# ZhengyiLuo/PHC

Measured on NVIDIA H100. Metric: env-steps/sec (fused obs+reward+PPO) at 4096 envs/GPU, higher is better.
Workload: dtype f32

## Files before the change

### include/phc_b200.h

```cpp
#ifndef PHC_B200_H_
#define PHC_B200_H_

#include <stdint.h>

#ifdef __cplusplus
extern "C" {
#endif

#if defined(_WIN32)
#define PHC_API __declspec(dllexport)
#else
#define PHC_API __attribute__((visibility("default")))
#endif

#define PHC_OK 0
#define PHC_ERR_INVALID_ARG (-1)
#define PHC_ERR_UNSUPPORTED (-2)
#define PHC_ERR_CUDA (-3)

PHC_API int phc_version(void);
PHC_API const char* phc_last_error(void);
PHC_API int64_t phc_launch_count(void);
PHC_API int phc_compiled_sm(void);

// ... 203 lines not shown
#define PHC_ACT_RELU_BITS 4
#define PHC_ACT_MASK_BITS 5
PHC_API int phc_gemm(const float* A, int64_t lda, int32_t a_kmajor, const float* B, int64_t ldb, int32_t b_kmajor, float* C,
             int64_t ldc, int32_t M, int32_t N, int32_t K, float alpha, const float* bias, int32_t act,
             float* aux, int64_t ldaux, int32_t accumulate, int32_t k_splits, void* stream);
PHC_API int phc_split_tf32(const float* x, int64_t ldx, int64_t rows, int32_t cols, float* hi, float* lo, int64_t ldo, void* stream);
PHC_API int phc_gemm_tc5(const float* A_hi, const float* A_lo, int64_t lda, int32_t a_kmajor, const float* B_hi, const float* B_lo,
                 int64_t ldb, int32_t b_kmajor, float* C, float* C_hi ,
                 float* C_lo, int64_t ldc, int32_t M, int32_t N, int32_t K, float alpha, const float* bias, int32_t act,
                 float* aux, int64_t ldaux, int32_t accumulate, int32_t k_splits, void* stream);
#define PHC_GEMM_GROUP_MAX 8
typedef struct PhcGemmDesc {
  const float* A; int64_t lda; int32_t a_kmajor;
  const float* B; int64_t ldb; int32_t b_kmajor;
  float* C; int64_t ldc;
  int32_t M, N, K;
  float alpha;
  const float* bias;
  int32_t act;
  float* aux; int64_t ldaux;
  int32_t accumulate, k_splits;
  const float* B_lo;
  const float* B_img;
} PhcGemmDesc;
typedef struct PhcGemmImageDesc {
  const float* B; int64_t ldb; int32_t b_kmajor;
  int32_t N, K;
  float* img;
} PhcGemmImageDesc;
PHC_API int64_t phc_gemm_image_floats(int32_t N, int32_t K);
PHC_API int phc_gemm_make_images(const PhcGemmImageDesc* images, int32_t count, void* stream);
PHC_API int phc_split_lo(const float* x, float* lo, int64_t n, void* stream);
PHC_API int phc_gemm_group(const PhcGemmDesc* problems, int32_t count, void* stream);
PHC_API int phc_gemm_tc5s(const float* A, int64_t lda, int32_t a_kmajor, const float* B, int64_t ldb, int32_t b_kmajor, float* C,
                  int64_t ldc, int32_t M, int32_t N, int32_t K, float alpha, const float* bias, int32_t act,
                  float* aux, int64_t ldaux, int32_t accumulate, int32_t k_splits, void* stream);
#define PHC_GEMM_FP32_3XTF32 0
#define PHC_GEMM_TF32_SINGLE_PASS 1
PHC_API int phc_gemm_set_precision(int32_t mode);
PHC_API int phc_gemm_tc5s_set_ctas(int32_t ctas);
PHC_API int phc_gemm_tc5s_set_tile(int32_t width);
PHC_API int phc_gemm_tc5s_set_sched(int32_t mode);
PHC_API int phc_pd_targets(const float* actions, int64_t lda, int64_t n, int32_t num_dofs, int32_t num_actions,
                   const int32_t* dof_of_action, const float* offset, const float* scale, const uint8_t* zero_mask,
                   float* out, int64_t ldo, void* stream);
PHC_API int phc_colsum(const float* X, int64_t ld, int32_t M, int32_t N, float alpha, float* out, int32_t accumulate,
// ... 45 lines not shown
```

### phc_b200/_lib.py

```python
from __future__ import annotations

import ctypes as C
import os

_HERE = os.path.dirname(os.path.abspath(__file__))
LIB_PATH = os.environ.get("PHC_LIB_PATH") or os.path.join(_HERE, "lib", "libphc_b200.so")

PHC_FLAG_UPRIGHT = 1 << 0
PHC_FLAG_LOCAL_ROOT_OBS = 1 << 1
PHC_FLAG_ROOT_HEIGHT_OBS = 1 << 2
PHC_FLAG_POWER_REWARD = 1 << 3
PHC_FLAG_EARLY_TERM = 1 << 4
PHC_FLAG_NO_COLLISION = 1 << 5
PHC_FLAG_TERM_USE_MEAN = 1 << 6
PHC_FLAG_OBS_ONLY = 1 << 7
PHC_FLAG_REWARD_FROM_CACHE = 1 << 8
PHC_FLAG_ZERO_OUT_FAR = 1 << 9
PHC_FLAG_CYCLE_MOTION = 1 << 10
PHC_FLAG_NO_SPECIALISE = 1 << 11
PHC_FLAG_SUBSET_REWARD = 1 << 12
PHC_FLAG_TASK_OBS_KP = 1 << 13
PHC_FLAG_RECOVERY = 1 << 14
PHC_FLAG_AMP_CURRENT = 1 << 15
PHC_ACT_NONE, PHC_ACT_RELU, PHC_ACT_SILU, PHC_ACT_SILU_BWD, PHC_ACT_RELU_BITS, PHC_ACT_MASK_BITS = 0, 1, 2, 3, 4, 5
# ... 30 lines not shown
        ("num_envs", C.c_int32), ("time_steps", C.c_int32), ("dt", C.c_float), ("traj_dt", C.c_float),
        ("flags", C.c_uint32),
        ("k_pos", C.c_float), ("k_rot", C.c_float), ("k_vel", C.c_float), ("k_ang_vel", C.c_float),
        ("w_pos", C.c_float), ("w_rot", C.c_float), ("w_vel", C.c_float), ("w_ang_vel", C.c_float),
        ("power_coef", C.c_float), ("term_thresh", C.c_float * PHC_MAX_BODIES), ("term_dist_mean", C.c_float),
        ("ext_parent", C.c_int32 * PHC_MAX_EXT_BODIES), ("ext_pos", (C.c_float * 3) * PHC_MAX_EXT_BODIES),
        ("num_key_bodies", C.c_int32), ("key_bodies", C.c_int32 * PHC_MAX_KEY_BODIES),
        ("amp_joints", C.c_int32 * PHC_MAX_AMP_JOINTS), ("num_amp_joints", C.c_int32),
        ("obs", _p), ("obs_stride", C.c_int64), ("rew", _p), ("reward_raw", _p), ("reset", _p), ("terminate", _p),
        ("amp_out", _p), ("amp_hist_in", _p), ("amp_out_stride", C.c_int64), ("amp_steps", C.c_int32),
        ("ref_body_pos", _p), ("ref_body_rot", _p), ("ref_body_vel", _p), ("ref_body_ang_vel", _p),
        ("ref_cache", _p),
        ("close_distance", C.c_float), ("far_distance", C.c_float), ("max_episode_length", C.c_int32), ("point_goal", _p),
        ("cycle_phase", _p), ("mpjpe", _p), ("body_pos_gt", _p), ("ring_head", _p),
        ("num_track", C.c_int32), ("track_slot", C.c_int8 * PHC_MAX_BODIES), ("occlusion", _p), ("shape_params", _p), ("num_shape", C.c_int32),
        ("limb_weights", _p), ("num_limb", C.c_int32), ("recovery_counter", _p),
    ]


class PhcGemmDesc(C.Structure):
    _fields_ = [("A", _p), ("lda", C.c_int64), ("a_kmajor", C.c_int32), ("B", _p), ("ldb", C.c_int64), ("b_kmajor", C.c_int32),
                ("C", _p), ("ldc", C.c_int64), ("M", C.c_int32), ("N", C.c_int32), ("K", C.c_int32), ("alpha", C.c_float),
                ("bias", _p), ("act", C.c_int32), ("aux", _p), ("ldaux", C.c_int64), ("accumulate", C.c_int32), ("k_splits", C.c_int32),
                ("B_lo", _p), ("B_img", _p)]


class PhcGemmImageDesc(C.Structure):
    _fields_ = [("B", _p), ("ldb", C.c_int64), ("b_kmajor", C.c_int32), ("N", C.c_int32), ("K", C.c_int32), ("img", _p)]


class PhcColsumDesc(C.Structure):
    _fields_ = [("X", _p), ("ld", C.c_int64), ("M", C.c_int32), ("N", C.c_int32), ("alpha", C.c_float), ("out", _p)]


PHC_GEMM_GROUP_MAX = 8
PHC_GEMM_FP32_3XTF32, PHC_GEMM_TF32_SINGLE_PASS = 0, 1

SIGNATURES = {
    "phc_version": (C.c_int, []),
    "phc_last_error": (C.c_char_p, []),
    "phc_compiled_sm": (C.c_int, []),
    "phc_launch_count": (C.c_int64, []),
    "phc_env_motion_gather": (C.c_int, [C.POINTER(PhcMotionLib), _p, C.c_int64, _p, _p]),
    "phc_motion_body_stride": (C.c_int, [C.c_int32]),
    "phc_reset_bookkeeping": (C.c_int, [_p, _p, _p, C.c_int64, _p, _p, _p, _p, _p, _p, _p, _p]),
    "phc_motion_dof_stride": (C.c_int, [C.c_int32]),
    "phc_motion_pack_dofs": (C.c_int, [_p, _p, C.c_int64, C.c_int32, _p, _p]),
# ... 91 lines not shown
```

### phc_b200/csrc/gemm_wgmma.cu

```cuda
#include <cuda_runtime.h>
#include <stdint.h>
#include <stdlib.h>
#include <string.h>

#include <type_traits>

#include "../../include/phc_b200.h"
#include "phc_common.cuh"

extern "C" void phc_set_error(const char* msg);
extern "C" int phc_check_cuda(cudaError_t e, const char* what);
extern "C" void phc_count_launches(int n);

namespace phc {
namespace wg {

constexpr int BM = 128, NUM_THREADS = 256, MAX_PROBLEMS = PHC_GEMM_GROUP_MAX;

template <int BN>
struct Cfg {
  static constexpr int BK = BN == 128 ? 32 : 16;
  static constexpr int A_TILE = BM * BK * 4;
  static constexpr int B_TILE = BN * BK * 4;
  static constexpr int STAGE = 2 * (A_TILE + B_TILE);
  static constexpr int STAGES = 3;
  static constexpr int SMEM = STAGES * STAGE;
  static constexpr int SBO = BK * 32;
  static constexpr int A_PER = BM * BK / NUM_THREADS;
  static constexpr int B_PER = BN * BK / NUM_THREADS;
};

constexpr int IMG_ROWS = 128, IMG_BK = 32, IMG_HALF = IMG_ROWS * IMG_BK, IMG_BLOCK = 2 * IMG_HALF;
constexpr int IMG_STAGES = 4;

struct Prob {
  const float* A; const float* B; const float* A_lo; const float* B_lo;
  const float* B_img;
  float* C; float* C_hi; float* C_lo;
  const float* bias;
  float* aux;
  long long lda, ldb, ldc, ldaux;
  int M, N, K;
  float alpha;
  int act, accumulate, a_k, b_k, k_splits;
  int tiles_m, tiles_n, kb_total, kb_per, tile_begin, tile_count;
  unsigned int* turn;
  int turn_first, turn_total;
};

struct Params {
  Prob p[MAX_PROBLEMS];
  int count, total_tiles;
  unsigned int* sched;
};

__device__ __forceinline__ void wgmma_tf32_n128(float (&d)[64], uint64_t da, uint64_t db) {
  asm volatile(
      "{\n\t.reg .pred p;\n\tsetp.ne.b32 p, 1, 0;\n\t"
      "wgmma.mma_async.sync.aligned.m64n128k8.f32.tf32.tf32 {%0, %1, %2, %3, %4, %5, %6, %7, %8, %9, %10, %11, %12, %13, %14, %15, %16, %17, %18, %19, %20, %21, %22, %23, %24, %25, %26, %27, %28, %29, %30, %31, %32, %33, %34, %35, %36, %37, %38, %39, %40, %41, %42, %43, %44, %45, %46, %47, %48, %49, %50, %51, %52, %53, %54, %55, %56, %57, %58, %59, %60, %61, %62, %63}, %64, %65, p, 1, 1;\n\t}"
      : "+f"(d[0]), "+f"(d[1]), "+f"(d[2]), "+f"(d[3]), "+f"(d[4]), "+f"(d[5]), "+f"(d[6]), "+f"(d[7]), "+f"(d[8]), "+f"(d[9]), "+f"(d[10]), "+f"(d[11]), "+f"(d[12]), "+f"(d[13]), "+f"(d[14]), "+f"(d[15]), "+f"(d[16]), "+f"(d[17]), "+f"(d[18]), "+f"(d[19]), "+f"(d[20]), "+f"(d[21]), "+f"(d[22]), "+f"(d[23]), "+f"(d[24]), "+f"(d[25]), "+f"(d[26]), "+f"(d[27]), "+f"(d[28]), "+f"(d[29]), "+f"(d[30]), "+f"(d[31]), "+f"(d[32]), "+f"(d[33]), "+f"(d[34]), "+f"(d[35]), "+f"(d[36]), "+f"(d[37]), "+f"(d[38]), "+f"(d[39]), "+f"(d[40]), "+f"(d[41]), "+f"(d[42]), "+f"(d[43]), "+f"(d[44]), "+f"(d[45]), "+f"(d[46]), "+f"(d[47]), "+f"(d[48]), "+f"(d[49]), "+f"(d[50]), "+f"(d[51]), "+f"(d[52]), "+f"(d[53]), "+f"(d[54]), "+f"(d[55]), "+f"(d[56]), "+f"(d[57]), "+f"(d[58]), "+f"(d[59]), "+f"(d[60]), "+f"(d[61]), "+f"(d[62]), "+f"(d[63])
// ... 140 lines not shown
        sts32(s_hi + o, hi(u[j]));
        if (MODE == 0) sts32(s_lo + o, split_lo(u[j]));
        if (MODE == 2) sts32(s_lo + o, ul[j]);
      }
    }
  }
}

__device__ __forceinline__ void split_rna(float x, float& h, float& l) {
  uint32_t a, b;
  asm("cvt.rna.tf32.f32 %0, %1;" : "=r"(a) : "f"(x));
  const float res = x - __uint_as_float(a);
  asm("cvt.rna.tf32.f32 %0, %1;" : "=r"(b) : "f"(res));
  h = __uint_as_float(a); l = __uint_as_float(b);
}

template <int BN, bool PRESPLIT, bool SINGLE>
__global__ void __launch_bounds__(NUM_THREADS, 1) gemm_wgmma_kernel(const __grid_constant__ Params P) {
  static_assert(!(PRESPLIT && SINGLE), "the pre-split operands are for the 3xTF32 products");
  using C = Cfg<BN>;
  constexpr int BK = C::BK;
  constexpr int MODE = SINGLE ? 1 : PRESPLIT ? 2 : 0;
  constexpr bool HAS_IMG = BN == IMG_ROWS && BK == IMG_BK && !PRESPLIT && !SINGLE;
  extern __shared__ __align__(128) uint8_t smem[];
  __shared__ int s_tile;
  __shared__ __align__(8) uint64_t s_bar[IMG_STAGES];
  const int tid = threadIdx.x, lane = tid & 31, wgi = tid >> 7, wq = (tid >> 5) & 3;
  const uint32_t sbase = (uint32_t)__cvta_generic_to_shared(smem);
  const uint32_t bar0 = (uint32_t)__cvta_generic_to_shared(s_bar);
  const bool dyn = P.sched != nullptr;
  int ring = 0;
  if constexpr (HAS_IMG) {
    if (tid == 0) {
#pragma unroll
      for (int s = 0; s < IMG_STAGES; ++s) mbar_init(bar0 + 8 * s, 1);
      mbar_init_fence();
    }
    __syncthreads();
  }

  for (int it = 0;; ++it) {
    int t;
    if (dyn) {
      if (tid == 0) s_tile = (int)atomicAdd(P.sched, 1u);
      __syncthreads();
      t = s_tile;
      __syncthreads();
    } else {
      t = blockIdx.x + it * gridDim.x;
    }
    if (t >= P.total_tiles) break;
    int gi = 0;
#pragma unroll 1
    while (gi + 1 < P.count && t >= P.p[gi].tile_begin + P.p[gi].tile_count) ++gi;
    const Prob& q = P.p[gi];
    const int tl = t - q.tile_begin;
    const int ni = tl % q.tiles_n, rr = tl / q.tiles_n, mi = rr % q.tiles_m, z = rr / q.tiles_m;
    const int m0 = mi * BM, n0 = ni * BN;
    const int kb_begin = z * q.kb_per;
    const int nkb = max(0, min(q.kb_total, kb_begin + q.kb_per) - kb_begin);
    if (nkb == 0) continue;
    const bool ak = q.a_k != 0, bk = q.b_k != 0;

    float acc[BN / 2];
#pragma unroll
    for (int j = 0; j < BN / 2; ++j) acc[j] = 0.f;
    bool staged = true;
    if constexpr (HAS_IMG) {
      if (q.B_img != nullptr) {
        staged = false;
        const int r = m0 + wgi * 64 + wq * 16 + (lane >> 2), c = lane & 3;
        const bool ok0 = r < q.M, ok1 = r + 8 < q.M;
        const float* arow0 = q.A + (long long)(ok0 ? r : 0) * q.lda + c;
        const float* arow1 = q.A + (long long)(ok1 ? r + 8 : 0) * q.lda + c;
        float ar[16];
        auto load_a = [&](int j) {
          const int k0 = (kb_begin + j) * BK;
          const bool full = k0 + BK <= q.K;
#pragma unroll
          for (int e = 0; e < 16; ++e) {
            const int k = k0 + 8 * (e >> 2) + 4 * ((e >> 1) & 1);
            const bool ok = ((e & 1) ? ok1 : ok0) && (full || k + c < q.K);
            ar[e] = ok ? ((e & 1) ? arow1 : arow0)[k] : 0.f;
          }
        };
        uint32_t ah[2][BK / 8][4], al[2][SINGLE ? 1 : BK / 8][4];
        constexpr uint32_t B_BYTES = (SINGLE ? 1 : 2) * IMG_HALF * 4, SLOT = 2 * IMG_HALF * 4;
        const float* img = q.B_img + (long long)ni * q.kb_total * IMG_BLOCK;
        auto issue = [&](int j) {
          const int s = (ring + j) % IMG_STAGES;
          mbar_expect_tx(bar0 + 8 * s, B_BYTES);
          bulk_g2s(sbase + s * SLOT, img + (long long)(kb_begin + j) * IMG_BLOCK, B_BYTES, bar0 + 8 * s);
// ... 38 lines not shown
          if (tid == 0 && j >= 1 && j - 1 + IMG_STAGES < nkb) issue(j - 1 + IMG_STAGES);
        };
#pragma unroll 1
        for (int j = 0; j < nkb; j += 2) {
          step(j, std::integral_constant<int, 0>());
          if (j + 1 < nkb) step(j + 1, std::integral_constant<int, 1>());
        }
        wgmma_wait<0>();
        ring += nkb;
      }
    }
    if (staged) {
      struct Regs { float a[C::A_PER], b[C::B_PER], a_lo[PRESPLIT ? C::A_PER : 1], b_lo[PRESPLIT ? C::B_PER : 1]; };
      Regs v;
      auto load = [&](int j) {
        const int k0 = (kb_begin + j) * BK;
        load_op<BM, BK>(v.a, q.A, q.lda, ak, m0, q.M, k0, q.K, tid);
        load_op<BN, BK>(v.b, q.B, q.ldb, bk, n0, q.N, k0, q.K, tid);
        if constexpr (PRESPLIT) {
          load_op<BM, BK>(v.a_lo, q.A_lo, q.lda, ak, m0, q.M, k0, q.K, tid);
          load_op<BN, BK>(v.b_lo, q.B_lo, q.ldb, bk, n0, q.N, k0, q.K, tid);
        }
      };
      auto stage = [&](int j) { return sbase + (uint32_t)((j % C::STAGES) * C::STAGE); };
      auto store = [&](int j) {
        const uint32_t s = stage(j);
        if constexpr (PRESPLIT) {
          store_op<BM, BK, C::A_PER, MODE>(v.a, v.a_lo, s, s + C::A_TILE, ak, tid);
          store_op<BN, BK, C::B_PER, MODE>(v.b, v.b_lo, s + 2 * C::A_TILE, s + 2 * C::A_TILE + C::B_TILE, bk, tid);
        } else {
          store_op<BM, BK, C::A_PER, MODE>(v.a, v.a, s, s + C::A_TILE, ak, tid);
          store_op<BN, BK, C::B_PER, MODE>(v.b, v.b, s + 2 * C::A_TILE, s + 2 * C::A_TILE + C::B_TILE, bk, tid);
        }
        fence_async_smem();
      };
      auto mma = [&](int j) {
        const uint32_t s = stage(j);
        const uint32_t a_hi = s + (uint32_t)(wgi * 8 * C::SBO), a_lo = a_hi + C::A_TILE;
        const uint32_t b_hi = s + 2 * C::A_TILE, b_lo = b_hi + C::B_TILE;
        wgmma_fence();
  #pragma unroll
        for (int kk = 0; kk < BK / 8; ++kk) {
          const uint32_t o = (uint32_t)kk * 256u;
          const uint64_t dAh = smem_desc(a_hi + o, 128, C::SBO), dBh = smem_desc(b_hi + o, 128, C::SBO);
          if constexpr (!SINGLE) {
            wgmma_tf32<BN>(acc, smem_desc(a_lo + o, 128, C::SBO), dBh);
            wgmma_tf32<BN>(acc, dAh, smem_desc(b_lo + o, 128, C::SBO));
          }
          wgmma_tf32<BN>(acc, dAh, dBh);
        }
        wgmma_commit();
      };
      load(0);
      store(0);
      if (nkb > 1) load(1);
      __syncthreads();
  #pragma unroll 1
      for (int j = 0; j < nkb; ++j) {
        mma(j);
        if (j + 1 < nkb) store(j + 1);
        if (j + 2 < nkb) load(j + 2);
        wgmma_wait<1>();
        __syncthreads();
      }
      wgmma_wait<0>();
    }
    __syncthreads();

    const bool ordered = q.turn != nullptr;
    volatile unsigned int* turn = ordered ? q.turn + mi * q.tiles_n + ni : nullptr;
    if (ordered) {
      if (tid == 0) {
        while (*turn != (unsigned)(q.turn_first + z)) __nanosleep(64);
        __threadfence();
      }
      __syncthreads();
    }
    const int act = q.act;
    const float* bias = (q.bias && z == 0) ? q.bias : nullptr;
#pragma unroll
    for (int h = 0; h < 2; ++h) {
      const int m = m0 + wgi * 64 + wq * 16 + (lane >> 2) + 8 * h;
      const bool row_ok = m < q.M;
      float* crow = q.C + (long long)m * q.ldc;
      float* arow = (q.aux && act < PHC_ACT_RELU_BITS && row_ok) ? q.aux + (long long)m * q.ldaux : nullptr;
      uint32_t* brow = (q.aux && act >= PHC_ACT_RELU_BITS && row_ok) ? reinterpret_cast<uint32_t*>(q.aux) + (long long)m * q.ldaux : nullptr;
#pragma unroll
      for (int qc = 0; qc < BN / 32; ++qc) {
        const int nb = n0 + 32 * qc;
        if (nb >= q.N) break;
        const uint32_t mbits = (act == PHC_ACT_MASK_BITS && brow) ? brow[nb >> 5] : 0u;
        uint32_t bits = 0;
#pragma unroll
        for (int jj = 0; jj < 4; ++jj) {
          const int j = 4 * qc + jj;
          const int nl = 8 * jj + 2 * (lane & 3);
          float v[2];
#pragma unroll
          for (int c = 0; c < 2; ++c) {
            const int n = nb + nl + c;
            float x = q.alpha * acc[4 * j + 2 * h + c];
            if (bias && n < q.N) x += bias[n];
            if (act == PHC_ACT_RELU || act == PHC_ACT_RELU_BITS) x = fmaxf(x, 0.f);
            if (act == PHC_ACT_RELU_BITS) bits |= (x > 0.f ? 1u : 0u) << (nl + c);
            else if (act == PHC_ACT_MASK_BITS) x = ((mbits >> (nl + c)) & 1u) ? x : 0.f;
            else if (arow && n < q.N) {
              if (act == PHC_ACT_SILU) { arow[n] = x; x = silu_f(x); }
              else if (act == PHC_ACT_SILU_BWD) x *= silu_grad_f(arow[n]);
              else x = arow[n] > 0.f ? x : 0.f;
            } else if (act == PHC_ACT_SILU) {
              x = silu_f(x);
            }
            v[c] = x;
          }
          if (!row_ok) continue;
          const int n = nb + nl;
          if (ordered) {
            if (n < q.N) crow[n] = __ldcg(crow + n) + v[0];
            if (n + 1 < q.N) crow[n + 1] = __ldcg(crow + n + 1) + v[1];
          } else if (q.accumulate) {
            if (n < q.N) atomicAdd(crow + n, v[0]);
            if (n + 1 < q.N) atomicAdd(crow + n + 1, v[1]);
          } else if (n + 1 < q.N) {
            *reinterpret_cast<float2*>(crow + n) = make_float2(v[0], v[1]);
          } else if (n < q.N) {
            crow[n] = v[0];
          }
          if (PRESPLIT && q.C_hi) {
            float h0, l0, h1, l1;
            split_rna(v[0], h0, l0); split_rna(v[1], h1, l1);
            if (n < q.N) { q.C_hi[(long long)m * q.ldc + n] = h0; q.C_lo[(long long)m * q.ldc + n] = l0; }
            if (n + 1 < q.N) { q.C_hi[(long long)m * q.ldc + n + 1] = h1; q.C_lo[(long long)m * q.ldc + n + 1] = l1; }
          }
        }
        if (act == PHC_ACT_RELU_BITS) {
          bits |= __shfl_xor_sync(0xffffffffu, bits, 1);
          bits |= __shfl_xor_sync(0xffffffffu, bits, 2);
          if (brow && (lane & 3) == 0) brow[nb >> 5] = bits;
        }
      }
    }
    if (ordered) {
// ... 46 lines not shown
        v[e] = (n < J.N && k + e < J.K) ? (J.b_k ? J.B[(long long)n * J.ldb + k + e] : J.B[(long long)(k + e) * J.ldb + n]) : 0.f;
      hi[c] = make_float4(trunc_hi(v[0]), trunc_hi(v[1]), trunc_hi(v[2]), trunc_hi(v[3]));
      lo[c] = make_float4(split_lo(v[0]), split_lo(v[1]), split_lo(v[2]), split_lo(v[3]));
    }
  }
}

static long long image_blocks(int N, int K) { return (long long)((N + IMG_ROWS - 1) / IMG_ROWS) * ((K + IMG_BK - 1) / IMG_BK); }

static int g_single_pass = 0;
static int g_tile = 0;
static int g_sched = -1;
constexpr int SCHED_SLOTS = 64;
__device__ unsigned int g_sched_counters[SCHED_SLOTS][2];
constexpr int TURN_SLOTS = 16, TURN_TILES = 8192;
__device__ unsigned int g_turns[TURN_SLOTS][TURN_TILES];

static int num_sms() {
  static int n = 0;
  if (!n) { int dev = 0; cudaGetDevice(&dev); cudaDeviceGetAttribute(&n, cudaDevAttrMultiProcessorCount, dev); if (n <= 0) n = 132; }
  return n;
}

static int add_problem(Params& P, int n, int tiles, int bn, const float* A, const float* A_lo, long long lda, int a_k, const float* B,
                       const float* B_lo, const float* B_img, long long ldb, int b_k, float* Cm, float* C_hi, float* C_lo, long long ldc, int M, int N, int K,
                       float alpha, const float* bias, int act, float* aux, long long ldaux, int accumulate, int k_splits) {
  const int bk = bn == 128 ? Cfg<128>::BK : Cfg<256>::BK;
  Prob& q = P.p[n];
  q.A = A; q.A_lo = A_lo; q.B = B; q.B_lo = B_lo; q.B_img = bn == IMG_ROWS ? B_img : nullptr; q.C = Cm; q.C_hi = C_hi; q.C_lo = C_lo; q.bias = bias; q.aux = aux;
  q.lda = lda; q.ldb = ldb; q.ldc = ldc; q.ldaux = ldaux; q.M = M; q.N = N; q.K = K; q.alpha = alpha; q.act = act;
  q.accumulate = accumulate ? 1 : 0; q.a_k = a_k ? 1 : 0; q.b_k = b_k ? 1 : 0;
  int ks = k_splits < 1 ? 1 : k_splits;
  q.tiles_m = (M + BM - 1) / BM;
  q.tiles_n = (N + bn - 1) / bn;
  q.kb_total = (K + bk - 1) / bk;
  if (ks > q.kb_total) ks = q.kb_total;
  q.kb_per = (q.kb_total + ks - 1) / ks;
  ks = (q.kb_total + q.kb_per - 1) / q.kb_per;
  q.k_splits = ks;
  q.turn = nullptr;
  q.tile_begin = tiles;
  q.tile_count = q.tiles_m * q.tiles_n * ks;
  return q.tile_count;
}

template <int BN, bool PRESPLIT, bool SINGLE>
static int launch_kernel(const Params& P, cudaStream_t stream) {
  static bool smem_set = false;
  if (!smem_set) {
    cudaError_t e = cudaFuncSetAttribute(gemm_wgmma_kernel<BN, PRESPLIT, SINGLE>, cudaFuncAttributeMaxDynamicSharedMemorySize, Cfg<BN>::SMEM);
    if (e != cudaSuccess) return phc_check_cuda(e, "cudaFuncSetAttribute(gemm_wgmma)");
    smem_set = true;
// ... 69 lines not shown
  }
  if constexpr (PRESPLIT) return launch_kernel<BN, true, false>(P, stream);
  return single ? launch_kernel<BN, false, true>(P, stream) : launch_kernel<BN, false, false>(P, stream);
}

}
}

static int validate_group(const PhcGemmDesc* d, int32_t count) {
  using namespace phc::wg;
  if (!d || count < 1 || count > MAX_PROBLEMS) { phc_set_error("phc_gemm_group: 1 <= count <= PHC_GEMM_GROUP_MAX problems"); return PHC_ERR_INVALID_ARG; }
  for (int i = 0; i < count; ++i) {
    const PhcGemmDesc& g = d[i];
    if (!g.A || !g.B || !g.C || g.M < 0 || g.N < 0 || g.K < 1) { phc_set_error("phc_gemm_group: bad problem (NULL operand or negative size)"); return PHC_ERR_INVALID_ARG; }
    if (g.M == 0 || g.N == 0) continue;
    if ((g.lda & 3) || (g.ldb & 3) || (g.ldc & 3)) { phc_set_error("phc_gemm_group: leading dimensions must be multiples of 4 floats (16-byte operand loads)"); return PHC_ERR_INVALID_ARG; }
    for (const void* p : {(const void*)g.A, (const void*)g.B, (const void*)g.C})
      if (reinterpret_cast<uintptr_t>(p) & 15) { phc_set_error("phc_gemm_group: A, B, C must be 16-byte aligned"); return PHC_ERR_INVALID_ARG; }
    const int ks = g.k_splits < 1 ? 1 : g.k_splits;
    if (g.act < 0 || g.act > PHC_ACT_MASK_BITS || ((g.act == PHC_ACT_SILU_BWD || g.act == PHC_ACT_MASK_BITS) && !g.aux)) { phc_set_error("phc_gemm_group: bad activation code"); return PHC_ERR_INVALID_ARG; }
    if (g.act >= PHC_ACT_RELU_BITS && g.aux && ((reinterpret_cast<uintptr_t>(g.aux) & 3) || g.ldaux < (g.N + 31) / 32)) { phc_set_error("phc_gemm_group: bit-mask aux needs ldaux >= ceil(N / 32) words"); return PHC_ERR_INVALID_ARG; }
    if (ks > 1 && (!g.accumulate || g.act || g.aux)) { phc_set_error("phc_gemm_group: split-K needs accumulate=1 and a linear epilogue"); return PHC_ERR_INVALID_ARG; }
    if (g.B_lo && (reinterpret_cast<uintptr_t>(g.B_lo) & 15)) { phc_set_error("phc_gemm_group: B_lo must be 16-byte aligned"); return PHC_ERR_INVALID_ARG; }
    if (g.B_img && ((reinterpret_cast<uintptr_t>(g.B_img) & 15) || !g.a_kmajor)) { phc_set_error("phc_gemm_group: B_img must be 16-byte aligned and comes with a_kmajor only"); return PHC_ERR_INVALID_ARG; }
  }
  auto span = [](const PhcGemmDesc& g, uintptr_t& lo, uintptr_t& hi) {
    lo = reinterpret_cast<uintptr_t>(g.C);
    hi = lo + (uintptr_t)(((int64_t)g.M - 1) * g.ldc + g.N) * sizeof(float);
  };
  for (int i = 0; i < count; ++i) {
    const PhcGemmDesc& a = d[i];
    if (a.M == 0 || a.N == 0) continue;
    uintptr_t a0, a1;
    span(a, a0, a1);
    for (int j = 0; j < i; ++j) {
      const PhcGemmDesc& b = d[j];
      if (b.M == 0 || b.N == 0) continue;
      uintptr_t b0, b1;
      span(b, b0, b1);
      if (a0 >= b1 || b0 >= a1) continue;
      if (a.accumulate && b.accumulate && a.C == b.C && a.M == b.M && a.N == b.N && a.ldc == b.ldc) continue;
      phc_set_error("phc_gemm_group: two problems write overlapping C ranges (only accumulating problems on the same C with the same M, N, ldc may)");
      return PHC_ERR_INVALID_ARG;
    }
  }
  return PHC_OK;
}

extern "C" int phc_gemm_group(const PhcGemmDesc* d, int32_t count, void* stream) {
  using namespace phc::wg;
  const int vrc = validate_group(d, count);
  if (vrc != PHC_OK) return vrc;
  if (g_sched < 0) { const char* v = getenv("PHC_TC5S_SCHED"); g_sched = (v && v[0] == 's') ? 0 : 1; }
  const int bn = g_tile == 256 ? 256 : 128;
  static Params P;
  memset(&P, 0, sizeof(P));
  int tiles = 0, n = 0;
  for (int i = 0; i < count; ++i) {
    const PhcGemmDesc& g = d[i];
    if (g.M == 0 || g.N == 0) continue;
    tiles += add_problem(P, n, tiles, bn, g.A, nullptr, g.lda, g.a_kmajor, g.B, nullptr, g.B_img, g.ldb, g.b_kmajor, g.C, nullptr, nullptr, g.ldc,
                         g.M, g.N, g.K, g.alpha, g.bias, g.act, g.aux, g.ldaux, g.accumulate, g.k_splits);
    ++n;
  }
  if (n == 0) return PHC_OK;
  P.count = n; P.total_tiles = tiles;
  cudaStream_t st = static_cast<cudaStream_t>(stream);
  const bool single = g_single_pass != 0;
  return bn == 256 ? launch<256, false>(P, g_sched == 1, single, st) : launch<128, false>(P, g_sched == 1, single, st);
}

extern "C" int phc_gemm_tc5s(const float* A, int64_t lda, int32_t a_kmajor, const float* B, int64_t ldb, int32_t b_kmajor, float* C,
                             int64_t ldc, int32_t M, int32_t N, int32_t K, float alpha, const float* bias, int32_t act, float* aux,
                             int64_t ldaux, int32_t accumulate, int32_t k_splits, void* stream) {
  PhcGemmDesc d;
  d.A = A; d.lda = lda; d.a_kmajor = a_kmajor; d.B = B; d.ldb = ldb; d.b_kmajor = b_kmajor; d.C = C; d.ldc = ldc;
  d.M = M; d.N = N; d.K = K; d.alpha = alpha; d.bias = bias; d.act = act; d.aux = aux; d.ldaux = ldaux;
  d.accumulate = accumulate; d.k_splits = k_splits; d.B_lo = nullptr; d.B_img = nullptr;
  return phc_gemm_group(&d, 1, stream);
}

extern "C" int phc_gemm_tc5(const float* A_hi, const float* A_lo, int64_t lda, int32_t a_kmajor, const float* B_hi,
                            const float* B_lo, int64_t ldb, int32_t b_kmajor, float* C, float* C_hi, float* C_lo, int64_t ldc,
                            int32_t M, int32_t N, int32_t K, float alpha, const float* bias, int32_t relu, float* mask,
                            int64_t ldmask, int32_t accumulate, int32_t k_splits, void* stream) {
  using namespace phc::wg;
  if (!A_hi || !A_lo || !B_hi || !B_lo || !C || M < 0 || N < 0 || K < 1) { phc_set_error("phc_gemm_tc5: bad arguments"); return PHC_ERR_INVALID_ARG; }
  if (M == 0 || N == 0) return PHC_OK;
  if ((lda & 3) || (ldb & 3) || (ldc & 1)) { phc_set_error("phc_gemm_tc5: lda, ldb must be multiples of 4 floats, ldc of 2"); return PHC_ERR_INVALID_ARG; }
  for (const void* p : {(const void*)A_hi, (const void*)A_lo, (const void*)B_hi, (const void*)B_lo})
    if (reinterpret_cast<uintptr_t>(p) & 15) { phc_set_error("phc_gemm_tc5: operands must be 16-byte aligned"); return PHC_ERR_INVALID_ARG; }
  if (reinterpret_cast<uintptr_t>(C) & 7) { phc_set_error("phc_gemm_tc5: C must be 8-byte aligned"); return PHC_ERR_INVALID_ARG; }
  if (k_splits < 1) k_splits = 1;
  if (relu < 0 || relu > PHC_ACT_SILU_BWD || (relu == PHC_ACT_SILU_BWD && !mask)) { phc_set_error("phc_gemm_tc5: bad activation code"); return PHC_ERR_INVALID_ARG; }
  if (k_splits > 1 && (!accumulate || relu || mask)) { phc_set_error("phc_gemm_tc5: split-K needs accumulate=1 and a linear epilogue"); return PHC_ERR_INVALID_ARG; }
  if ((C_hi == nullptr) != (C_lo == nullptr) || (C_hi && accumulate)) { phc_set_error("phc_gemm_tc5: C_hi/C_lo come as a pair and not with accumulate"); return PHC_ERR_INVALID_ARG; }
  static Params P;
  memset(&P, 0, sizeof(P));
  P.total_tiles = add_problem(P, 0, 0, 128, A_hi, A_lo, lda, a_kmajor, B_hi, B_lo, nullptr, ldb, b_kmajor, C, C_hi, C_lo, ldc, M, N, K, alpha, bias,
                              relu, mask, ldmask, accumulate, k_splits);
  P.count = 1;
  return launch<128, true>(P, false, false, static_cast<cudaStream_t>(stream));
}

extern "C" int phc_split_tf32(const float* x, int64_t ldx, int64_t rows, int32_t cols, float* hi, float* lo, int64_t ldo,
                              void* stream) {
  if (!x || !hi || !lo || rows < 0 || cols < 1 || ldx < cols || ldo < cols) { phc_set_error("phc_split_tf32: bad arguments"); return PHC_ERR_INVALID_ARG; }
  if (rows == 0) return PHC_OK;
  int64_t g = (rows * cols + 255) / 256; if (g > 132 * 8) g = 132 * 8;
  phc::wg::split_tf32_kernel<<<(unsigned)g, 256, 0, static_cast<cudaStream_t>(stream)>>>(x, ldx, rows, cols, hi, lo, ldo);
  phc_count_launches(1);
  return phc_check_cuda(cudaGetLastError(), "split_tf32_kernel");
}

extern "C" int64_t phc_gemm_image_floats(int32_t N, int32_t K) {
  return N < 1 || K < 1 ? 0 : phc::wg::image_blocks(N, K) * phc::wg::IMG_BLOCK;
}

extern "C" int phc_gemm_make_images(const PhcGemmImageDesc* d, int32_t count, void* stream) {
  using namespace phc::wg;
  if (count < 0 || (count > 0 && !d)) { phc_set_error("phc_gemm_make_images: bad arguments"); return PHC_ERR_INVALID_ARG; }
  for (int i = 0; i < count; ++i) {
// ... 58 lines not shown
```

### phc_b200/learning/amp_agent.py

```python
from __future__ import annotations

import copy
import os
import time
from typing import Dict, Optional

import torch

from .. import _lib, ops
from ..ops import _ptr, _stream
from . import dist as D
from .networks import AMPNetwork, MLPEngine, round4

DEFAULT_CONFIG = dict(
    name="Humanoid", multi_gpu=False, normalize_input=True, normalize_value=True, normalize_advantage=True,
    gamma=0.99, tau=0.95, learning_rate=2e-5, truncate_grads=True, grad_norm=50.0, e_clip=0.2, horizon_length=32,
    minibatch_size=16384, mini_epochs=6, critic_coef=5.0, clip_value=False, bounds_loss_coef=10.0, entropy_coef=0.0,
    amp_obs_demo_buffer_size=200000, amp_replay_buffer_size=200000, amp_replay_keep_prob=0.01, amp_batch_size=512,
    amp_minibatch_size=4096, disc_coef=5.0, disc_logit_reg=0.01, disc_grad_penalty=5.0, disc_reward_scale=2.0,
    disc_weight_decay=0.0001, normalize_amp_input=True, task_reward_w=0.5, disc_reward_w=0.5, max_epochs=10000000,
    save_frequency=2500, save_best_after=100, seed=0,
    network=dict(mlp=dict(units=[1024, 512], activation="relu"), disc=dict(units=[1024, 512], activation="relu"),
                 sigma_init=-2.9),
)
# ... 692 lines not shown
                        dw, dx = eng.bwd_descs(stk, li, xin, ws)
                        descs += [dw, dx]
                        l = stk.layers[li]
                        dY = ws["dout"] if li == len(stk.layers) - 1 else ws["dh"][li]
                        sums.append((dY, dY.shape[0], l.out_dim, net.bias(l, grad=True)))
                after = None
                if k < len(gp):
                    gdescs, after = gp[k]
                    descs += gdescs
                eng.run_group(descs)
                eng.colsum_group(sums)
                if after is not None:
                    after()
            head = net.disc.head
            _lib.check(lib.phc_axpy2d(net.weight(head).data_ptr(), head.in_pad, net.weight(head, True).data_ptr(), head.in_pad, 1,
                                      head.in_dim, 2.0 * self._disc_coef * self._disc_logit_reg, self._stats[11:].data_ptr(), st))
            if self._disc_weight_decay != 0:
                for l in net.disc.layers:
                    _lib.check(lib.phc_axpy2d(net.weight(l).data_ptr(), l.in_pad, net.weight(l, True).data_ptr(), l.in_pad, l.out_dim,
                                              l.in_dim, 2.0 * self._disc_coef * self._disc_weight_decay, self._stats[12:].data_ptr(), st))

    def _gp_steps(self, x_demo: torch.Tensor, Bd: int, st):
        lib, net, eng = self._lib, self.model, self.engine
        from .networks import group_splits
        hid, head = net.disc.hidden, net.disc.head
        L = len(hid)
        ws = self._ws_disc
        h_demo = [h[2 * Bd:3 * Bd] for h in ws["h"]]
        bits = [hb[2 * Bd:3 * Bd] for hb in ws["hbits"]] if "hbits" in ws else None
        mask = lambda i: dict(act=_lib.PHC_ACT_MASK_BITS, aux=bits[i]) if bits is not None else dict(aux=h_demo[i])
        u, e, g = self._gp_u, self._gp_e, self._gp_g
        _lib.check(lib.phc_relu_mask_row(h_demo[L - 1].data_ptr(), h_demo[L - 1].stride(0), net.weight(head).data_ptr(), Bd,
                                         hid[L - 1].out_dim, u[L - 1].data_ptr(), u[L - 1].stride(0), st))
        steps = []
        for li in range(L - 1, 0, -1):
            l = hid[li]
            steps.append(([eng.gdesc(u[li], True, net.weight(l), False, u[li - 1], Bd, l.in_dim, l.out_dim, B_img=eng.image(l, False),
                                     **mask(li - 1))], None))
        l0 = hid[0]
        c = self._disc_coef * self._disc_grad_penalty

        def penalty():
            _lib.check(lib.phc_scale_sumsq(g.data_ptr(), g.stride(0), Bd, l0.in_dim, 2.0 * c / Bd, self._stats[10:].data_ptr(), st))
        steps.append(([eng.gdesc(u[0], True, net.weight(l0), False, g, Bd, l0.in_dim, l0.out_dim, B_img=eng.image(l0, False))], penalty))
        for li in range(L):
            l = hid[li]
            src = g if li == 0 else e[li - 1]
            after = None
            if li == L - 1:
                after = lambda: eng.colsum(e[L - 1], Bd, hid[L - 1].out_dim, net.weight(head, True))
            steps.append(([eng.gdesc(u[li], False, src, False, net.weight(l, True), l.out_dim, l.in_dim, Bd, accumulate=True, k_splits=group_splits(Bd)),
                           eng.gdesc(src, True, net.weight(l), True, e[li], Bd, l.out_dim, l.in_dim, B_img=eng.image(l, True), **mask(li))],
                          after))
        return steps

    def _disc_grad_penalty_backward(self, x_demo: torch.Tensor, h_demo, Bd: int) -> None:
        lib, net, eng, st = self._lib, self.model, self.engine, _stream()
        hid = net.disc.hidden
        L = len(hid)
        head = net.disc.head
        u, e = self._gp_u, self._gp_e
        _lib.check(lib.phc_relu_mask_row(h_demo[L - 1].data_ptr(), h_demo[L - 1].stride(0), net.weight(head).data_ptr(), Bd,
                                         hid[L - 1].out_dim, u[L - 1].data_ptr(), u[L - 1].stride(0), st))
        for li in range(L - 1, 0, -1):
            l = hid[li]
            eng.gemm(u[li], True, net.weight(l), False, u[li - 1], Bd, l.in_dim, l.out_dim, mask=h_demo[li - 1])
        l0 = hid[0]
        eng.gemm(u[0], True, net.weight(l0), False, self._gp_g, Bd, l0.in_dim, l0.out_dim)
        c = self._disc_coef * self._disc_grad_penalty
        _lib.check(lib.phc_scale_sumsq(self._gp_g.data_ptr(), self._gp_g.stride(0), Bd, l0.in_dim, 2.0 * c / Bd,
                                       self._stats[10:].data_ptr(), st))
        tiles = lambda l: ((l.out_dim + 127) // 128) * ((l.in_dim + 127) // 128)
        from .networks import _splits
        eng.gemm(u[0], False, self._gp_g, False, net.weight(l0, True), l0.out_dim, l0.in_dim, Bd, accumulate=True,
# ... 151 lines not shown
```

### phc_b200/learning/networks.py

```python
from __future__ import annotations

import math
import os
from dataclasses import dataclass
from typing import Dict, List, Optional, Sequence, Tuple

import torch

from .. import _lib
from ..ops import _ptr, _stream


def round4(x: int) -> int:
    return (x + 3) & ~3


@dataclass
class LinearSpec:
    name: str
    in_dim: int
    out_dim: int
    w_off: int = 0
    b_off: int = 0
    img_fwd: int = 0
# ... 164 lines not shown
    env = os.environ.get("PHC_DW_KB_PER_SPLIT")
    per = int(env) if env else 32
    return int(max(1, min(64, round(((K + 31) // 32) / per))))


class MLPEngine:

    _mode_set = None

    def __init__(self, net: AMPNetwork, backend: Optional[str] = None, precision: str = "fp32"):
        assert precision in ("fp32", "tf32")
        self.precision = precision
        self.net = net
        self.lib = _lib.load()
        self.dev = net.device
        self._ws: Dict[Tuple[str, int], Dict[str, torch.Tensor]] = {}
        self.backend = backend or os.environ.get("PHC_GEMM", "tc5s")
        assert self.backend in ("mma", "tc5", "tc5s")
        if precision == "tf32" and self.backend != "tc5s":
            raise ValueError("precision='tf32' (single tensor-core pass) exists on the tc5s back end only")
        self._companions: Dict[Tuple[int, Tuple[int, ...], Tuple[int, ...]], Tuple[torch.Tensor, torch.Tensor]] = {}
        self.gemm_flops = 0.0
        self.uses_images = self.backend == "tc5s" and precision == "fp32"
        if self.backend == "tc5":
            net.refresh_split()

    def companions(self, t: torch.Tensor) -> Tuple[torch.Tensor, torch.Tensor]:
        key = (t.data_ptr(), tuple(t.shape), tuple(t.stride()))
        c = self._companions.get(key)
        if c is None:
            base_rows, ld = t.shape[0], t.stride(0)
            c = (torch.zeros(base_rows, ld, device=self.dev)[:, :t.shape[1]], torch.zeros(base_rows, ld, device=self.dev)[:, :t.shape[1]])
            self._companions[key] = c
        return c

    def split(self, t: torch.Tensor) -> Tuple[torch.Tensor, torch.Tensor]:
        hi, lo = self.companions(t)
        rc = self.lib.phc_split_tf32(t.data_ptr(), t.stride(0), t.shape[0], t.shape[1], hi.data_ptr(), lo.data_ptr(), hi.stride(0), _stream())
        if rc:
            _lib.check(rc, "phc_split_tf32")
        return hi, lo

    def _weight_parts(self, W: torch.Tensor) -> Optional[Tuple[torch.Tensor, torch.Tensor]]:
        p = self.net.params
        off = (W.data_ptr() - p.data_ptr()) // 4
        if 0 <= off < p.numel() and W.data_ptr() >= p.data_ptr():
# ... 37 lines not shown
        return _lib.PhcGemmDesc(A.data_ptr(), A.stride(0), 1 if a_k else 0, B.data_ptr(), B.stride(0), 1 if b_k else 0, C.data_ptr(),
                                C.stride(0), M, N, K, alpha, _ptr(bias), act, _ptr(aux), aux.stride(0) if aux is not None else 0,
                                1 if accumulate else 0, k_splits, None, _ptr(B_img))

    def fwd_desc(self, st: MLPStack, li: int, x: torch.Tensor, ws: Dict[str, torch.Tensor]):
        net, l, B = self.net, st.layers[li], x.shape[0]
        inp = x if li == 0 else ws["h"][li - 1]
        silu = st.activation == "silu"
        if li < len(st.hidden):
            out = ws["h"][li]
            act = _lib.PHC_ACT_SILU if silu else (_lib.PHC_ACT_RELU_BITS if "hbits" in ws else _lib.PHC_ACT_RELU)
            aux = ws["z"][li] if silu else (ws["hbits"][li] if "hbits" in ws else None)
        else:
            out = ws["out"]
            act = _lib.PHC_ACT_NONE if not st.head_relu else (_lib.PHC_ACT_SILU if silu else (_lib.PHC_ACT_RELU_BITS if "obits" in ws else _lib.PHC_ACT_RELU))
            aux = None if not st.head_relu else (ws["z_out"] if silu else ws.get("obits"))
        return self.gdesc(inp, True, net.weight(l), True, out, B, l.out_dim, l.in_dim, bias=net.bias(l), act=act, aux=aux,
                          B_img=self.image(l, True))

    def bwd_descs(self, st: MLPStack, li: int, x: torch.Tensor, ws: Dict[str, torch.Tensor], dx: Optional[torch.Tensor] = None):
        net, l, B = self.net, st.layers[li], x.shape[0]
        dY = ws["dout"] if li == len(st.layers) - 1 else ws["dh"][li]
        inp = x if li == 0 else ws["h"][li - 1]
        dw = self.gdesc(dY, False, inp, False, net.weight(l, grad=True), l.out_dim, l.in_dim, B, accumulate=True, k_splits=group_splits(B))
        dxd = None
        img = self.image(l, False)
        if li > 0:
            if st.activation == "silu":
                dxd = self.gdesc(dY, True, net.weight(l), False, ws["dh"][li - 1], B, l.in_dim, l.out_dim, act=_lib.PHC_ACT_SILU_BWD, aux=ws["z"][li - 1], B_img=img)
            elif "hbits" in ws:
                dxd = self.gdesc(dY, True, net.weight(l), False, ws["dh"][li - 1], B, l.in_dim, l.out_dim, act=_lib.PHC_ACT_MASK_BITS, aux=ws["hbits"][li - 1], B_img=img)
            else:
                dxd = self.gdesc(dY, True, net.weight(l), False, ws["dh"][li - 1], B, l.in_dim, l.out_dim, aux=ws["h"][li - 1], B_img=img)
        elif dx is not None:
            dxd = self.gdesc(dY, True, net.weight(l), False, dx, B, l.in_dim, l.out_dim, B_img=img)
        return dw, dxd

    def _set_mode(self) -> None:
        mode = _lib.PHC_GEMM_TF32_SINGLE_PASS if self.precision == "tf32" else _lib.PHC_GEMM_FP32_3XTF32
        if MLPEngine._mode_set != mode:
            _lib.check(self.lib.phc_gemm_set_precision(mode), "phc_gemm_set_precision")
            MLPEngine._mode_set = mode

    def run_group(self, descs) -> None:
        self._set_mode()
        descs = [d for d in descs if d is not None]
        for i in range(0, len(descs), _lib.PHC_GEMM_GROUP_MAX):
            part = descs[i:i + _lib.PHC_GEMM_GROUP_MAX]
            self.gemm_flops += sum(2.0 * d.M * d.N * d.K for d in part)
            arr = (_lib.PhcGemmDesc * len(part))(*part)
            rc = self.lib.phc_gemm_group(arr, len(part), _stream())
            if rc:
                _lib.check(rc, "phc_gemm_group")

    def forward_group(self, items) -> None:
        depth = max(len(st.layers) for st, _, _ in items)
        for li in range(depth):
            self.run_group([self.fwd_desc(st, li, x, ws) for st, x, ws in items if li < len(st.layers)])

    def colsum(self, X, M, N, out, alpha=1.0, accumulate=True):
        rc = self.lib.phc_colsum(X.data_ptr(), X.stride(0), M, N, alpha, out.data_ptr(), 1 if accumulate else 0, _stream())
        if rc:
            _lib.check(rc, "phc_colsum")

    def colsum_group(self, items) -> None:
        for i in range(0, len(items), _lib.PHC_GEMM_GROUP_MAX):
            part = items[i:i + _lib.PHC_GEMM_GROUP_MAX]
            arr = (_lib.PhcColsumDesc * len(part))(*[_lib.PhcColsumDesc(X.data_ptr(), X.stride(0), M, N, 1.0, out.data_ptr()) for X, M, N, out in part])
            rc = self.lib.phc_colsum_group(arr, len(part), _stream())
            if rc:
                _lib.check(rc, "phc_colsum_group")
# ... 77 lines not shown
```

Baseline: 219,500.

## Pre-split activations into TMA images for large weight-gradient GEMMs

Adds an A_img path: for large weight-gradient GEMMs, both operands are converted into pre-split hi/lo image blocks and fed through a bulk-copy plus mbarrier multistage pipeline. This replaces per-thread loads and in-kernel splitting. The image conversion is an extra kernel per group, cached by pointer. The ordered split-K epilogue now also loads old C values up front instead of interleaving each load with its store.

```diff
diff --git a/include/phc_b200.h b/include/phc_b200.h
--- a/include/phc_b200.h
+++ b/include/phc_b200.h
@@ -249,6 +249,7 @@
   int32_t accumulate, k_splits;
   const float* B_lo;
   const float* B_img;
+  const float* A_img;
 } PhcGemmDesc;
 typedef struct PhcGemmImageDesc {
   const float* B; int64_t ldb; int32_t b_kmajor;
diff --git a/phc_b200/_lib.py b/phc_b200/_lib.py
--- a/phc_b200/_lib.py
+++ b/phc_b200/_lib.py
@@ -76,7 +76,7 @@
     _fields_ = [("A", _p), ("lda", C.c_int64), ("a_kmajor", C.c_int32), ("B", _p), ("ldb", C.c_int64), ("b_kmajor", C.c_int32),
                 ("C", _p), ("ldc", C.c_int64), ("M", C.c_int32), ("N", C.c_int32), ("K", C.c_int32), ("alpha", C.c_float),
                 ("bias", _p), ("act", C.c_int32), ("aux", _p), ("ldaux", C.c_int64), ("accumulate", C.c_int32), ("k_splits", C.c_int32),
-                ("B_lo", _p), ("B_img", _p)]
+                ("B_lo", _p), ("B_img", _p), ("A_img", _p)]
 
 
 class PhcGemmImageDesc(C.Structure):
diff --git a/phc_b200/csrc/gemm_wgmma.cu b/phc_b200/csrc/gemm_wgmma.cu
--- a/phc_b200/csrc/gemm_wgmma.cu
+++ b/phc_b200/csrc/gemm_wgmma.cu
@@ -36,6 +36,7 @@
 struct Prob {
   const float* A; const float* B; const float* A_lo; const float* B_lo;
   const float* B_img;
+  const float* A_img;
   float* C; float* C_hi; float* C_lo;
   const float* bias;
   float* aux;
@@ -222,18 +223,24 @@
   constexpr int BK = C::BK;
   constexpr int MODE = SINGLE ? 1 : PRESPLIT ? 2 : 0;
   constexpr bool HAS_IMG = BN == IMG_ROWS && BK == IMG_BK && !PRESPLIT && !SINGLE;
+  static_assert(!HAS_IMG || (C::A_TILE == IMG_HALF * 4 && C::B_TILE == IMG_HALF * 4), "an image block pair is one stage");
   extern __shared__ __align__(128) uint8_t smem[];
   __shared__ int s_tile;
   __shared__ __align__(8) uint64_t s_bar[IMG_STAGES];
+  __shared__ __align__(8) uint64_t s_pbar[C::STAGES];
   const int tid = threadIdx.x, lane = tid & 31, wgi = tid >> 7, wq = (tid >> 5) & 3;
   const uint32_t sbase = (uint32_t)__cvta_generic_to_shared(smem);
   const uint32_t bar0 = (uint32_t)__cvta_generic_to_shared(s_bar);
+  const uint32_t pbar0 = (uint32_t)__cvta_generic_to_shared(s_pbar);
   const bool dyn = P.sched != nullptr;
   int ring = 0;
+  uint32_t pphase = 0;
   if constexpr (HAS_IMG) {
     if (tid == 0) {
 #pragma unroll
       for (int s = 0; s < IMG_STAGES; ++s) mbar_init(bar0 + 8 * s, 1);
+#pragma unroll
+      for (int s = 0; s < C::STAGES; ++s) mbar_init(pbar0 + 8 * s, 1);
       mbar_init_fence();
     }
     __syncthreads();
@@ -265,9 +272,50 @@
     float acc[BN / 2];
 #pragma unroll
     for (int j = 0; j < BN / 2; ++j) acc[j] = 0.f;
+    auto stage = [&](int j) { return sbase + (uint32_t)((j % C::STAGES) * C::STAGE); };
+    auto mma = [&](int j) {
+      const uint32_t s = stage(j);
+      const uint32_t a_hi = s + (uint32_t)(wgi * 8 * C::SBO), a_lo = a_hi + C::A_TILE;
+      const uint32_t b_hi = s + 2 * C::A_TILE, b_lo = b_hi + C::B_TILE;
+      wgmma_fence();
+#pragma unroll
+      for (int kk = 0; kk < BK / 8; ++kk) {
+        const uint32_t o = (uint32_t)kk * 256u;
+        const uint64_t dAh = smem_desc(a_hi + o, 128, C::SBO), dBh = smem_desc(b_hi + o, 128, C::SBO);
+        if constexpr (!SINGLE) {
+          wgmma_tf32<BN>(acc, smem_desc(a_lo + o, 128, C::SBO), dBh);
+          wgmma_tf32<BN>(acc, dAh, smem_desc(b_lo + o, 128, C::SBO));
+        }
+        wgmma_tf32<BN>(acc, dAh, dBh);
+      }
+      wgmma_commit();
+    };
     bool staged = true;
     if constexpr (HAS_IMG) {
-      if (q.B_img != nullptr) {
+      if (q.A_img != nullptr) {
+        staged = false;
+        const float* aimg = q.A_img + (long long)mi * q.kb_total * IMG_BLOCK;
+        const float* bimg = q.B_img + (long long)ni * q.kb_total * IMG_BLOCK;
+        auto issue = [&](int j) {
+          const uint32_t s = stage(j), bar = pbar0 + 8 * (j % C::STAGES);
+          mbar_expect_tx(bar, C::STAGE);
+          bulk_g2s(s, aimg + (long long)(kb_begin + j) * IMG_BLOCK, IMG_BLOCK * 4, bar);
+          bulk_g2s(s + 2 * C::A_TILE, bimg + (long long)(kb_begin + j) * IMG_BLOCK, IMG_BLOCK * 4, bar);
+        };
+        if (tid == 0)
+          for (int j = 0; j < min(nkb, C::STAGES); ++j) issue(j);
+#pragma unroll 1
+        for (int j = 0; j < nkb; ++j) {
+          const int s = j % C::STAGES;
+          mbar_wait(pbar0 + 8 * s, (pphase >> s) & 1u);
+          pphase ^= 1u << s;
+          mma(j);
+          wgmma_wait<1>();
+          __syncthreads();
+          if (tid == 0 && j >= 1 && j + 2 < nkb) issue(j + 2);
+        }
+        wgmma_wait<0>();
+      } else if (q.B_img != nullptr) {
         staged = false;
         const int r = m0 + wgi * 64 + wq * 16 + (lane >> 2), c = lane & 3;
         const bool ok0 = r < q.M, ok1 = r + 8 < q.M;
@@ -352,7 +400,6 @@
           load_op<BN, BK>(v.b_lo, q.B_lo, q.ldb, bk, n0, q.N, k0, q.K, tid);
         }
       };
-      auto stage = [&](int j) { return sbase + (uint32_t)((j % C::STAGES) * C::STAGE); };
       auto store = [&](int j) {
         const uint32_t s = stage(j);
         if constexpr (PRESPLIT) {
@@ -363,23 +410,6 @@
           store_op<BN, BK, C::B_PER, MODE>(v.b, v.b, s + 2 * C::A_TILE, s + 2 * C::A_TILE + C::B_TILE, bk, tid);
         }
         fence_async_smem();
-      };
-      auto mma = [&](int j) {
-        const uint32_t s = stage(j);
-        const uint32_t a_hi = s + (uint32_t)(wgi * 8 * C::SBO), a_lo = a_hi + C::A_TILE;
-        const uint32_t b_hi = s + 2 * C::A_TILE, b_lo = b_hi + C::B_TILE;
-        wgmma_fence();
-  #pragma unroll
-        for (int kk = 0; kk < BK / 8; ++kk) {
-          const uint32_t o = (uint32_t)kk * 256u;
-          const uint64_t dAh = smem_desc(a_hi + o, 128, C::SBO), dBh = smem_desc(b_hi + o, 128, C::SBO);
-          if constexpr (!SINGLE) {
-            wgmma_tf32<BN>(acc, smem_desc(a_lo + o, 128, C::SBO), dBh);
-            wgmma_tf32<BN>(acc, dAh, smem_desc(b_lo + o, 128, C::SBO));
-          }
-          wgmma_tf32<BN>(acc, dAh, dBh);
-        }
-        wgmma_commit();
       };
       load(0);
       store(0);
@@ -421,6 +451,14 @@
         if (nb >= q.N) break;
         const uint32_t mbits = (act == PHC_ACT_MASK_BITS && brow) ? brow[nb >> 5] : 0u;
         uint32_t bits = 0;
+        float old[8];
+        if (ordered && row_ok) {
+#pragma unroll
+          for (int e = 0; e < 8; ++e) {
+            const int n = nb + 8 * (e >> 1) + 2 * (lane & 3) + (e & 1);
+            old[e] = n < q.N ? __ldcg(crow + n) : 0.f;
+          }
+        }
 #pragma unroll
         for (int jj = 0; jj < 4; ++jj) {
           const int j = 4 * qc + jj;
@@ -446,8 +484,8 @@
           if (!row_ok) continue;
           const int n = nb + nl;
           if (ordered) {
-            if (n < q.N) crow[n] = __ldcg(crow + n) + v[0];
-            if (n + 1 < q.N) crow[n + 1] = __ldcg(crow + n + 1) + v[1];
+            if (n < q.N) crow[n] = old[2 * jj] + v[0];
+            if (n + 1 < q.N) crow[n + 1] = old[2 * jj + 1] + v[1];
           } else if (q.accumulate) {
             if (n < q.N) atomicAdd(crow + n, v[0]);
             if (n + 1 < q.N) atomicAdd(crow + n + 1, v[1]);
@@ -540,12 +578,13 @@
   return n;
 }
 
-static int add_problem(Params& P, int n, int tiles, int bn, const float* A, const float* A_lo, long long lda, int a_k, const float* B,
-                       const float* B_lo, const float* B_img, long long ldb, int b_k, float* Cm, float* C_hi, float* C_lo, long long ldc, int M, int N, int K,
+static int add_problem(Params& P, int n, int tiles, int bn, const float* A, const float* A_lo, const float* A_img, long long lda, int a_k,
+                       const float* B, const float* B_lo, const float* B_img, long long ldb, int b_k, float* Cm, float* C_hi, float* C_lo, long long ldc, int M, int N, int K,
                        float alpha, const float* bias, int act, float* aux, long long ldaux, int accumulate, int k_splits) {
   const int bk = bn == 128 ? Cfg<128>::BK : Cfg<256>::BK;
   Prob& q = P.p[n];
-  q.A = A; q.A_lo = A_lo; q.B = B; q.B_lo = B_lo; q.B_img = bn == IMG_ROWS ? B_img : nullptr; q.C = Cm; q.C_hi = C_hi; q.C_lo = C_lo; q.bias = bias; q.aux = aux;
+  q.A = A; q.A_lo = A_lo; q.B = B; q.B_lo = B_lo; q.B_img = bn == IMG_ROWS ? B_img : nullptr;
+  q.A_img = q.B_img ? A_img : nullptr; q.C = Cm; q.C_hi = C_hi; q.C_lo = C_lo; q.bias = bias; q.aux = aux;
   q.lda = lda; q.ldb = ldb; q.ldc = ldc; q.ldaux = ldaux; q.M = M; q.N = N; q.K = K; q.alpha = alpha; q.act = act;
   q.accumulate = accumulate ? 1 : 0; q.a_k = a_k ? 1 : 0; q.b_k = b_k ? 1 : 0;
   int ks = k_splits < 1 ? 1 : k_splits;
@@ -661,7 +700,8 @@
     if (g.act >= PHC_ACT_RELU_BITS && g.aux && ((reinterpret_cast<uintptr_t>(g.aux) & 3) || g.ldaux < (g.N + 31) / 32)) { phc_set_error("phc_gemm_group: bit-mask aux needs ldaux >= ceil(N / 32) words"); return PHC_ERR_INVALID_ARG; }
     if (ks > 1 && (!g.accumulate || g.act || g.aux)) { phc_set_error("phc_gemm_group: split-K needs accumulate=1 and a linear epilogue"); return PHC_ERR_INVALID_ARG; }
     if (g.B_lo && (reinterpret_cast<uintptr_t>(g.B_lo) & 15)) { phc_set_error("phc_gemm_group: B_lo must be 16-byte aligned"); return PHC_ERR_INVALID_ARG; }
-    if (g.B_img && ((reinterpret_cast<uintptr_t>(g.B_img) & 15) || !g.a_kmajor)) { phc_set_error("phc_gemm_group: B_img must be 16-byte aligned and comes with a_kmajor only"); return PHC_ERR_INVALID_ARG; }
+    if (g.A_img && ((reinterpret_cast<uintptr_t>(g.A_img) & 15) || !g.B_img)) { phc_set_error("phc_gemm_group: A_img must be 16-byte aligned and comes with B_img only"); return PHC_ERR_INVALID_ARG; }
+    if (g.B_img && ((reinterpret_cast<uintptr_t>(g.B_img) & 15) || (!g.a_kmajor && !g.A_img))) { phc_set_error("phc_gemm_group: B_img must be 16-byte aligned and comes with a_kmajor or A_img only"); return PHC_ERR_INVALID_ARG; }
   }
   auto span = [](const PhcGemmDesc& g, uintptr_t& lo, uintptr_t& hi) {
     lo = reinterpret_cast<uintptr_t>(g.C);
@@ -698,7 +738,7 @@
   for (int i = 0; i < count; ++i) {
     const PhcGemmDesc& g = d[i];
     if (g.M == 0 || g.N == 0) continue;
-    tiles += add_problem(P, n, tiles, bn, g.A, nullptr, g.lda, g.a_kmajor, g.B, nullptr, g.B_img, g.ldb, g.b_kmajor, g.C, nullptr, nullptr, g.ldc,
+    tiles += add_problem(P, n, tiles, bn, g.A, nullptr, g.A_img, g.lda, g.a_kmajor, g.B, nullptr, g.B_img, g.ldb, g.b_kmajor, g.C, nullptr, nullptr, g.ldc,
                          g.M, g.N, g.K, g.alpha, g.bias, g.act, g.aux, g.ldaux, g.accumulate, g.k_splits);
     ++n;
   }
@@ -715,7 +755,7 @@
   PhcGemmDesc d;
   d.A = A; d.lda = lda; d.a_kmajor = a_kmajor; d.B = B; d.ldb = ldb; d.b_kmajor = b_kmajor; d.C = C; d.ldc = ldc;
   d.M = M; d.N = N; d.K = K; d.alpha = alpha; d.bias = bias; d.act = act; d.aux = aux; d.ldaux = ldaux;
-  d.accumulate = accumulate; d.k_splits = k_splits; d.B_lo = nullptr; d.B_img = nullptr;
+  d.accumulate = accumulate; d.k_splits = k_splits; d.B_lo = nullptr; d.B_img = nullptr; d.A_img = nullptr;
   return phc_gemm_group(&d, 1, stream);
 }
 
@@ -736,7 +776,7 @@
   if ((C_hi == nullptr) != (C_lo == nullptr) || (C_hi && accumulate)) { phc_set_error("phc_gemm_tc5: C_hi/C_lo come as a pair and not with accumulate"); return PHC_ERR_INVALID_ARG; }
   static Params P;
   memset(&P, 0, sizeof(P));
-  P.total_tiles = add_problem(P, 0, 0, 128, A_hi, A_lo, lda, a_kmajor, B_hi, B_lo, nullptr, ldb, b_kmajor, C, C_hi, C_lo, ldc, M, N, K, alpha, bias,
+  P.total_tiles = add_problem(P, 0, 0, 128, A_hi, A_lo, nullptr, lda, a_kmajor, B_hi, B_lo, nullptr, ldb, b_kmajor, C, C_hi, C_lo, ldc, M, N, K, alpha, bias,
                               relu, mask, ldmask, accumulate, k_splits);
   P.count = 1;
   return launch<128, true>(P, false, false, static_cast<cudaStream_t>(stream));
diff --git a/phc_b200/learning/amp_agent.py b/phc_b200/learning/amp_agent.py
--- a/phc_b200/learning/amp_agent.py
+++ b/phc_b200/learning/amp_agent.py
@@ -738,7 +738,6 @@
 
     def _gp_steps(self, x_demo: torch.Tensor, Bd: int, st):
         lib, net, eng = self._lib, self.model, self.engine
-        from .networks import group_splits
         hid, head = net.disc.hidden, net.disc.head
         L = len(hid)
         ws = self._ws_disc
@@ -765,7 +764,7 @@
             after = None
             if li == L - 1:
                 after = lambda: eng.colsum(e[L - 1], Bd, hid[L - 1].out_dim, net.weight(head, True))
-            steps.append(([eng.gdesc(u[li], False, src, False, net.weight(l, True), l.out_dim, l.in_dim, Bd, accumulate=True, k_splits=group_splits(Bd)),
+            steps.append(([eng.dw_desc(u[li], src, net.weight(l, True), l.out_dim, l.in_dim, Bd),
                            eng.gdesc(src, True, net.weight(l), True, e[li], Bd, l.out_dim, l.in_dim, B_img=eng.image(l, True), **mask(li))],
                           after))
         return steps
diff --git a/phc_b200/learning/networks.py b/phc_b200/learning/networks.py
--- a/phc_b200/learning/networks.py
+++ b/phc_b200/learning/networks.py
@@ -210,6 +210,7 @@
         self._companions: Dict[Tuple[int, Tuple[int, ...], Tuple[int, ...]], Tuple[torch.Tensor, torch.Tensor]] = {}
         self.gemm_flops = 0.0
         self.uses_images = self.backend == "tc5s" and precision == "fp32"
+        self._act_images: Dict[Tuple[int, int, int, int], torch.Tensor] = {}
         if self.backend == "tc5":
             net.refresh_split()
 
@@ -293,7 +294,7 @@
         net, l, B = self.net, st.layers[li], x.shape[0]
         dY = ws["dout"] if li == len(st.layers) - 1 else ws["dh"][li]
         inp = x if li == 0 else ws["h"][li - 1]
-        dw = self.gdesc(dY, False, inp, False, net.weight(l, grad=True), l.out_dim, l.in_dim, B, accumulate=True, k_splits=group_splits(B))
+        dw = self.dw_desc(dY, inp, net.weight(l, grad=True), l.out_dim, l.in_dim, B)
         dxd = None
         img = self.image(l, False)
         if li > 0:
@@ -307,6 +308,32 @@
             dxd = self.gdesc(dY, True, net.weight(l), False, dx, B, l.in_dim, l.out_dim, B_img=img)
         return dw, dxd
 
+    def dw_desc(self, dY: torch.Tensor, X: torch.Tensor, dW: torch.Tensor, M: int, N: int, K: int):
+        d = self.gdesc(dY, False, X, False, dW, M, N, K, accumulate=True, k_splits=group_splits(K))
+        tm, tn = -(-M // 128), -(-N // 128)
+        if self.uses_images and tm * tn >= 4 * (tm + tn):
+            d.image_of = (dY, X)
+        return d
+
+    def make_images(self, descs):
+        jobs = {}
+        for d in descs:
+            srcs = getattr(d, "image_of", None)
+            if srcs is None:
+                continue
+            ptrs = []
+            for t, rows in zip(srcs, (d.M, d.N)):
+                key = (t.data_ptr(), t.stride(0), rows, d.K)
+                img = self._act_images.get(key)
+                if img is None:
+                    img = torch.empty(self.lib.phc_gemm_image_floats(rows, d.K), dtype=torch.float32, device=self.dev)
+                    self._act_images[key] = img
+                if key not in jobs:
+                    jobs[key] = _lib.PhcGemmImageDesc(t.data_ptr(), t.stride(0), 0, rows, d.K, img.data_ptr())
+                ptrs.append(img.data_ptr())
+            d.A_img, d.B_img = ptrs
+        return (_lib.PhcGemmImageDesc * len(jobs))(*jobs.values()), len(jobs)
+
     def _set_mode(self) -> None:
         mode = _lib.PHC_GEMM_TF32_SINGLE_PASS if self.precision == "tf32" else _lib.PHC_GEMM_FP32_3XTF32
         if MLPEngine._mode_set != mode:
@@ -318,6 +345,9 @@
         descs = [d for d in descs if d is not None]
         for i in range(0, len(descs), _lib.PHC_GEMM_GROUP_MAX):
             part = descs[i:i + _lib.PHC_GEMM_GROUP_MAX]
+            jobs, n = self.make_images(part)
+            if n:
+                _lib.check(self.lib.phc_gemm_make_images(jobs, n, _stream()), "phc_gemm_make_images")
             self.gemm_flops += sum(2.0 * d.M * d.N * d.K for d in part)
             arr = (_lib.PhcGemmDesc * len(part))(*part)
             rc = self.lib.phc_gemm_group(arr, len(part), _stream())
```

Result: faster. 231,400 (median of 6 runs) (+5.4%).
